# tyt0223/emqx

Measured on AMD Instinct MI355X. Metric: topics matched/sec (node) at 10M filters, 1/2/4/8 GPUs; % HBM roofline, higher is better.
Workload: dtype u32

## Files before the change

### emqx_amd/csrc/egm_ctx.h

```cpp
#pragma once
#include <hip/hip_runtime_api.h>
#include <string.h>

#include <algorithm>
#include <condition_variable>
#include <memory>
#include <mutex>
#include <new>
#include <string>
#include <thread>
#include <unordered_map>
#include <vector>

#include "../../include/emqx_gpu_match.h"
#include "egm_alloc.h"
#include "egm_buf.h"
#include "egm_kernels.h"
#include "egm_table.h"

#pragma GCC visibility push(hidden)
namespace egm {

struct StreamUses {
  std::vector<std::pair<hipStream_t, hipEvent_t>> v;
// ... 15 lines not shown
    }
    v.clear();
  }
};

struct PipeSlot {
  bool busy = false;
  bool waiting = false;
  bool held = false;
  bool sync = false;
  bool abandoned = false;
  uint32_t gen = 0;
  uint32_t n = 0;
  int mode = 0;
  bool want_packed = false;
  bool packed = false;
  uint64_t bytes = 0, maxlen = 0, cap = 0;
  uint64_t o_off = 0;
  PinBuf h_in, h_out, h_stats;
  DevBuf d_in, d_row, d_ids, d_flags, d_row32, d_pk;
  hipEvent_t ev_in = nullptr, ev_match = nullptr, ev_done = nullptr;
  uint64_t epoch = 0;
  uint64_t launch_gen = 0, copied_gen = 0;
  bool copy_failed = false;
  ~PipeSlot() {
    if (ev_in) hipEventDestroy(ev_in);
    if (ev_match) hipEventDestroy(ev_match);
    if (ev_done) hipEventDestroy(ev_done);
  }
};

struct OutLayout {
  size_t o_res, o_row, o_ids, o_fl, o_cnt, total;
};
inline size_t al16(size_t x) { return (x + 15) & ~(size_t)15; }
inline OutLayout out_layout(uint64_t n, uint64_t cap) {
  OutLayout o;
  o.o_res = sizeof(ResultHdr);
  o.o_row = al16(o.o_res + sizeof(egm_result));
  o.o_ids = al16(o.o_row + (n + 1) * 8);
  o.o_fl = al16(o.o_ids + cap * 4);
  o.o_cnt = al16(o.o_fl + n);
  o.total = o.o_cnt + n * 4 + 16;
  return o;
}

struct MatchWs {
  DevBuf wid, lv, tfl, cnt, ids_tmp, pieces, deferred, heavy_stack, tile_sums, stats;
  DevBuf skey, skey_out, sval, order, wfix, sort_tmp;
  DevBuf rec, chunks, dir;
  uint64_t pieces_cap = 0, ids_tmp_cap = 0, rec_cap = 0;
  uint32_t rec_grain = REC_GRAIN, flush_lim = 0;
  uint32_t heavy_cap = 0;
  hipEvent_t ev = nullptr;
  hipStream_t stream = nullptr;
  uint64_t used = 0;
  ~MatchWs() {
    if (ev) hipEventDestroy(ev);
  }
};
constexpr uint32_t MATCH_WORKSPACES = 2;

struct Slot {
  DevBuf nodes, hash_child, edges, dict, dict_blob, dict_off;
  uint64_t n_nodes = 0, n_hc = 0, n_edges = 0, n_dict = 0, n_blob = 0, n_off = 0;
  bool valid = false;
  DirtyLog pending;
  StreamUses uses;
  uint64_t bytes() const {
    return nodes.cap + hash_child.cap + edges.cap + dict.cap + dict_blob.cap + dict_off.cap;
  }
};

struct SubsState {
  bool built = false;
  std::vector<uint64_t> row;
  std::vector<uint32_t> subs;
  std::unordered_map<uint32_t, std::vector<uint32_t>> lists;
  std::unordered_map<uint32_t, uint4> recs;
  std::vector<uint32_t> pending;
  std::vector<uint32_t> stale[2];
  uint64_t tail = 0, garbage = 0;
  int cur = 0;
  StreamUses uses[2];
  uint64_t epoch = 0;
  uint64_t last_appended = 0, last_patched = 0;
  bool last_rebuilt = false;
};

struct Epoch {
  DevTable view{};
  int slot = 0;
  uint64_t id = 0;
  uint64_t n_filters = 0, n_nodes = 0, n_edges = 0, n_words = 0, bytes = 0;
  uint64_t fid_end = 0;
};

struct CommitStats {
  uint64_t h2d = 0, d2d = 0, patched = 0;
  double ms = 0;
};

struct Timing {
  struct Series {
    std::vector<hipEvent_t> ev;
    double ms = 0;
// ... 202 lines not shown
```

### emqx_amd/csrc/egm_kernels.h

```cpp
#pragma once
#include <hip/hip_runtime_api.h>
#include <stdint.h>

#include "egm_common.h"

namespace egm {

struct DevTable {
  const NodeRec* nodes;
  const uint32_t* hash_child;
  const EdgeSlot* edges;
  uint32_t edge_mask;
  const DictSlot* dict;
  uint32_t dict_mask;
  const uint8_t* dict_blob;
  const uint64_t* dict_off;
  uint32_t sig_packed;
};

struct MatchStats {
  unsigned long long cursor;
  unsigned long long visited;
  unsigned long long pieces;
  unsigned long long total_ids;
  unsigned int n_deferred;
  unsigned int heavy_next;
  unsigned int overflow;
  unsigned int errors;
  unsigned int guard;
  unsigned int slow_lanes;
  unsigned long long iters;
  unsigned long long popped;
  unsigned long long bounded;
  unsigned long long lit_probes;
  unsigned long long plus_reads;
  unsigned int n_deep;
  unsigned int slow_iters;
  unsigned long long rec_cursor;
};

constexpr uint32_t REC_HDR = 4;
constexpr uint32_t REC_IDS = REC_HDR + 32;
constexpr uint32_t REC_TAG = 0x5EC0u << 16;
constexpr uint32_t REC_JUMP = 0x4A4Du << 16;
constexpr uint32_t REC_GRAIN = 16384;
constexpr uint32_t REC_DIR = 64;
#ifndef EGM_REC_ALIGN
#define EGM_REC_ALIGN 32
#endif
__host__ __device__ constexpr uint32_t rec_size(uint32_t n_entries) {
  return (REC_IDS + n_entries + (EGM_REC_ALIGN - 1u)) & ~(EGM_REC_ALIGN - 1u);
}
constexpr uint32_t CHUNK_WALKED = 1u;
constexpr uint32_t CHUNK_HEAVY = 2u;

struct MatchWork {
  uint32_t* wid;
  uint32_t* lv;
  uint8_t* tfl;
  uint32_t* cnt;
  uint32_t walk_rows;
  uint32_t ct;
  uint32_t* rec;
  uint64_t rec_cap;
  uint32_t rec_grain;
  uint32_t flush_lim;
  uint4* chunks;
  uint32_t* dir;
  uint32_t* ids_tmp;
  uint64_t ids_cap;
  uint4* pieces;
  uint64_t pieces_cap;
  uint32_t* deferred;
  uint32_t* deep;
  uint4* heavy_stack;
  uint32_t heavy_waves;
  uint32_t heavy_cap;
  uint64_t* tile_sums;
  MatchStats* stats;
  uint32_t debug;
  uint32_t* skey;
  uint32_t* skey_out;
  uint64_t* sval;
  uint64_t* order;
  uint32_t* wfix;
  void* sort_tmp;
  size_t sort_tmp_bytes;
  uint32_t key_shape;
  const uint32_t* n_live;
};

constexpr uint32_t KEY_LEVELS = 4;
constexpr uint32_t FIX_WORDS = 8;
struct WalkOrderOut {
  uint32_t* key;
  uint64_t* val;
  uint32_t* wfix;
  uint32_t shape;
  const uint32_t* n_live;
};

constexpr uint32_t GUARD_STACK = 4u;
constexpr uint32_t GUARD_LOOP = 8u;

constexpr uint32_t DEBUG_FORCE_HEAVY = 1u;
constexpr uint32_t DEBUG_INPUT_ORDER = 4u;
constexpr uint32_t DEBUG_FORCE_GUARD = 8u;

uint32_t walk_key_bits(uint32_t shape);
size_t walk_sort_temp_bytes(uint32_t n, uint32_t shape);
hipError_t launch_walk_sort(uint32_t* keys, uint32_t* keys_tmp, uint64_t* vals, uint64_t* out, void* tmp,
                            MatchStats* stats, uint32_t n, uint32_t kbits, hipStream_t s);

struct MatchOut {
  uint64_t* row_ptr;
  uint32_t* ids;
  uint64_t ids_cap;
  uint32_t* topic;
};
// ... 55 lines not shown
                              hipStream_t s);

hipError_t launch_copy_out(const uint64_t* row, uint32_t n, const uint32_t* ids, uint64_t ids_cap,
                           const uint8_t* flags, uint8_t* h_row, uint8_t* h_ids, uint8_t* h_fl, hipStream_t s,
                           const MatchStats* st = nullptr, MatchStats* h_st = nullptr);

constexpr uint32_t PFX_TOPICS_MAX = 1u << 30;
struct PrefixSlots {
  uint32_t n_ranks, cap_topics;
  uint64_t cap_bytes;
  __host__ __device__ uint64_t off_offsets() const { return 16 + 4ull * cap_topics; }
  __host__ __device__ uint64_t off_bytes() const { return (off_offsets() + 4ull * (cap_topics + 1) + 15) & ~15ull; }
  __host__ __device__ uint64_t slot_bytes() const { return (off_bytes() + cap_bytes + 15) & ~15ull; }
};
hipError_t launch_prefix_route(const uint8_t* blob, const uint32_t* off, uint32_t n, const uint8_t* vpart_rank,
                               uint32_t n_vparts, const PrefixSlots& ps, uint8_t* send, unsigned long long* ctr,
                               uint64_t* dst, hipStream_t s);

hipError_t launch_patch(void* dst, uint32_t rec_bytes, const uint32_t* idx, const void* src, uint64_t n,
                        hipStream_t s);

constexpr uint32_t RN_TERM = 0x80000000u;
constexpr uint32_t RS_SINGLE = 0x80000000u;

struct RetainView {
  const uint4* nodes;
  const uint4* edges;
  uint32_t edge_mask;
  const uint32_t* msg;
  const uint64_t* expiry;
  uint32_t n_topics;
};

struct RetainWork {
  const uint32_t* off;
  const uint32_t* wid;
  const uint32_t* lv;
  const uint8_t* tfl;
  uint32_t* pc;
  uint32_t* paux;
  uint64_t* poff;
  uint64_t* tiles;
  uint32_t *rf, *rlo, *rhi;
  uint32_t* n_ranges;
  uint32_t range_cap;
  uint32_t* alive;
  uint64_t* apre;
  uint32_t* fcnt;
  uint32_t* roff;
  uint64_t now;
  int ge_plain;
};

hipError_t launch_tokenise(const DevTable& tab, const uint8_t* blob, const uint32_t* off, uint32_t n, uint32_t* wid,
                           uint32_t* lv, uint8_t* tfl, hipStream_t s);
hipError_t launch_rs_alive(const RetainView& v, const RetainWork& w, hipStream_t s);
hipError_t launch_rs_init(uint32_t n, uint32_t* pf, uint32_t* pn, hipStream_t s);
hipError_t launch_rs_level(const RetainView& v, const RetainWork& w, uint32_t level, uint32_t np,
                           const uint32_t* pf, const uint32_t* pn, hipStream_t s);
hipError_t launch_rs_fill(const RetainWork& w, uint32_t np, uint64_t nnext, const uint32_t* pf, uint32_t* pf2,
                          uint32_t* pn2, hipStream_t s);
hipError_t launch_rs_rows(const RetainWork& w, uint32_t nr, uint32_t n, uint64_t* row, hipStream_t s);
hipError_t launch_rs_expand(const RetainView& v, const RetainWork& w, uint32_t nr, const uint64_t* row,
                            uint32_t* ids, hipStream_t s);

}
```

### emqx_amd/csrc/egm_kernels.hip

```cpp
#include <hip/hip_runtime.h>

#include <stdio.h>
#include <stdlib.h>
#include <string.h>

#include <algorithm>

#include "egm_kernels.h"

namespace egm {

constexpr int MODE_TRIE = 0;
constexpr int MODE_ROUTES = 1;

constexpr int TOK_BLOCK = 256;
#ifndef EGM_TOK_LDS
#define EGM_TOK_LDS 16256
#endif
constexpr int TOK_LDS = EGM_TOK_LDS;
#ifndef EGM_TOK_WORDS
#define EGM_TOK_WORDS 2528
#endif
constexpr int TOK_WORDS = EGM_TOK_WORDS;
#ifndef EGM_TOK_U
#define EGM_TOK_U 2
#endif
constexpr int TOK_U = EGM_TOK_U;
constexpr int SCAN_TILE = 2048;


__device__ __forceinline__ uint32_t mbcnt(uint64_t m) {
  return __builtin_amdgcn_mbcnt_hi((uint32_t)(m >> 32), __builtin_amdgcn_mbcnt_lo((uint32_t)m, 0u));
}
__device__ __forceinline__ uint32_t popc(uint64_t m) { return (uint32_t)__popcll(m); }

__device__ __forceinline__ void wave_sync() {
  __builtin_amdgcn_fence(__ATOMIC_RELEASE, "wavefront");
  __builtin_amdgcn_s_waitcnt(0xC07F);
  __builtin_amdgcn_wave_barrier();
  __builtin_amdgcn_fence(__ATOMIC_ACQUIRE, "wavefront");
}

__device__ __forceinline__ uint32_t wave_excl_scan(uint32_t v, uint32_t lane, uint32_t* total) {
  uint32_t x = v;
#pragma unroll
  for (int d = 1; d < 64; d <<= 1) {
    uint32_t y = __shfl_up(x, d, 64);
    if (lane >= (uint32_t)d) x += y;
  }
  *total = __shfl(x, 63, 64);
  return x - v;
}

__device__ __forceinline__ uint4 ld16(const void* p) { return *(const uint4*)p; }

__device__ __forceinline__ uint32_t byte_of(uint4 v, uint32_t k) {
  uint32_t w = (k < 8) ? (k < 4 ? v.x : v.y) : (k < 12 ? v.z : v.w);
  return (w >> (8 * (k & 3))) & 0xFFu;
}

__device__ uint32_t dict_probe(const DevTable& tab, uint64_t h, const uint8_t* p, uint32_t len) {
  uint32_t i = (uint32_t)h & tab.dict_mask;
  for (;;) {
    const uint8_t* sp = (const uint8_t*)(tab.dict + i);
    const uint4 a = ld16(sp);
    const uint4 b = ld16(sp + 16);
    if (a.z == NONE) return WID_NONE;
    if (a.x == (uint32_t)h && a.y == (uint32_t)(h >> 32) && a.w == len) {
      bool eq = true;
      if (len <= 16) {
        for (uint32_t k = 0; k < len; ++k) eq &= byte_of(b, k) == p[k];
      } else {
        const uint8_t* q = tab.dict_blob + tab.dict_off[a.z];
        for (uint32_t k = 0; k < len; ++k) eq &= q[k] == p[k];
      }
      if (eq) return a.z;
// ... 53 lines not shown
  const uint32_t x = v ^ 0x2F2F2F2Fu;
  return (x - 0x01010101u) & ~x & 0x80808080u;
}

__device__ __forceinline__ uint32_t byte_range(uint32_t lo, uint32_t hi) {
  const uint32_t a = lo >= 4 ? 0u : (0xFFFFFFFFu << (8 * lo));
  const uint32_t b = hi >= 4 ? 0xFFFFFFFFu : ((1u << (8 * hi)) - 1u);
  return a & b;
}

__device__ __forceinline__ uint32_t dict_resolve(const DevTable& tab, uint64_t h, uint4 a, uint4 b,
                                                 const uint32_t* sw, uint32_t st, uint32_t len) {
  uint32_t i = (uint32_t)h & tab.dict_mask;
  for (;;) {
    if (a.z == NONE) return WID_NONE;
    if (a.x == (uint32_t)h && a.y == (uint32_t)(h >> 32) && a.w == len) {
      bool eq = true;
      if (len <= 16) {
        const uint32_t bw[4] = {b.x, b.y, b.z, b.w};
#pragma unroll
        for (uint32_t k = 0; k < 16; k += 4)
          if (k < len) eq &= low_bytes(lds_word(sw, st + k), len - k) == low_bytes(bw[k >> 2], len - k);
      } else {
        const uint8_t* q = tab.dict_blob + tab.dict_off[a.z];
        for (uint32_t k = 0; k < len; ++k) eq &= q[k] == lds_byte(sw, st + k);
      }
      if (eq) return a.z;
    }
    i = (i + 1) & tab.dict_mask;
    const uint8_t* sp = (const uint8_t*)(tab.dict + i);
    a = ld16(sp);
    b = ld16(sp + 16);
  }
}

__device__ __forceinline__ uint32_t walk_key(const uint32_t* w4, uint32_t D, uint32_t shape) {
  uint64_t h = FNV_BASIS;
  uint32_t k = 0, used = 0;
#pragma unroll
  for (uint32_t l = 0; l < KEY_LEVELS; ++l) {
    const uint32_t bl = (shape >> (4 * l)) & 0xFu;
    h = mix64((h ^ w4[l]) * FNV_PRIME);
    const uint32_t b = (l < D && bl) ? (uint32_t)(h >> (64 - bl)) : 0u;
    k = bl ? ((k << bl) | b) : k;
    used += bl;
  }
  return used < 32 ? k << (32 - used) : k;
}

__device__ __forceinline__ uint64_t sort_val(uint32_t t, uint32_t D, uint32_t f, bool fixed) {
  return (uint64_t)t | ((uint64_t)(min(D, 0xFFFFFFu) | ((f & 0x7Fu) << 24) | (fixed ? 0x80000000u : 0u)) << 32);
}

__global__ __launch_bounds__(TOK_BLOCK) void k_tokenise(DevTable tab, const uint8_t* __restrict__ blob,
                                                        const uint32_t* __restrict__ off, uint32_t n,
                                                        uint32_t* __restrict__ wid, uint32_t* __restrict__ lv,
                                                        uint8_t* __restrict__ tfl, WalkOrderOut wo) {
  __shared__ __attribute__((aligned(16))) uint32_t sw[TOK_LDS / 4 + 1];
  __shared__ uint32_t wpos[TOK_WORDS];
  __shared__ uint8_t wtop[TOK_WORDS];
  __shared__ uint32_t tg[TOK_BLOCK];
  __shared__ uint32_t tex[TOK_BLOCK];
  __shared__ uint32_t tflag[TOK_BLOCK];
  __shared__ uint32_t wsum[TOK_BLOCK / 64];
  const uint32_t blk0 = blockIdx.x * TOK_BLOCK;
  if (blk0 >= n) return;
  const uint32_t tid = threadIdx.x, lane = tid & 63, wv = tid >> 6;
  const uint32_t n_live = wo.n_live ? (wo.n_live[2] ? 0u : min(wo.n_live[0], n)) : n;
  const uint32_t tend = min(blk0 + (uint32_t)TOK_BLOCK, n);
  uint32_t S = TOK_BLOCK;
  for (uint32_t t0 = blk0; t0 < tend;) {
    uint32_t t1, sa, ea;
    for (;;) {
      t1 = min(t0 + S, tend);
      sa = off[t0] & ~3u;
      ea = (off[t1] + 3u) & ~3u;
      if ((ea - sa) <= (uint32_t)TOK_LDS || S == 1) break;
      S >>= 1;
    }
    const uint32_t t = t0 + tid;
    if ((ea - sa) > (uint32_t)TOK_LDS) {
      if (tid == 0) {
        const uint32_t ts = off[t0], len = off[t0 + 1] - ts;
        uint32_t l;
        uint8_t fl;
        tokenise_one(tab, (const uint32_t*)(blob + (ts & ~3u)), ts & 3u, len, ts + t0, wid, &l, &fl);
        if (t0 >= n_live) fl |= TF_SKIP;
        lv[t0] = l;
        tfl[t0] = fl;
        if (wo.key) {
          wo.key[t0] = 0xFFFFFFFFu;
          wo.val[t0] = sort_val(t0, l, fl, false);
        }
      }
      t0 = t1;
      continue;
    }
    {
      const uint32_t nw = (ea - sa) >> 2;
      const uint32_t* src = (const uint32_t*)(blob + sa);
      for (uint32_t i = tid; i < nw; i += TOK_BLOCK) sw[i] = src[i];
    }
    __syncthreads();

    uint32_t ts = 0, len = 0, D = 0, fl = 0;
    if (t < t1) {
      ts = off[t] - sa;
      len = off[t + 1] - off[t];
      uint32_t c = 0;
      for (uint32_t q = ts & ~3u; q < ts + len; q += 4) {
        const uint32_t lo = q < ts ? ts - q : 0u, hi = min(4u, ts + len - q);
        c += popc((uint64_t)(slash_mask(sw[q >> 2]) & byte_range(lo, hi)));
      }
      D = c + 1;
      if (len > 0 && lds_byte(sw, ts) == '$') fl |= TF_DOLLAR;
      if (t >= n_live) fl |= TF_SKIP;
    }
    uint32_t wtot;
    uint32_t ex = wave_excl_scan(D, lane, &wtot);
    if (lane == 0) wsum[wv] = wtot;
    __syncthreads();
    uint32_t W = 0;
#pragma unroll
    for (int k = 0; k < TOK_BLOCK / 64; ++k) {
      if ((uint32_t)k < wv) ex += wsum[k];
      W += wsum[k];
    }
    __syncthreads();
    if (W > (uint32_t)TOK_WORDS) {
      if (S > 1) {
        S >>= 1;
        continue;
      }
      if (tid == 0) {
        uint32_t l;
        uint8_t f;
        tokenise_one(tab, sw, ts, len, off[t] + t, wid, &l, &f);
        if (t >= n_live) f |= TF_SKIP;
        lv[t] = l;
        tfl[t] = f;
        if (wo.key) {
          wo.key[t] = 0xFFFFFFFFu;
          wo.val[t] = sort_val(t, l, f, false);
        }
      }
      __syncthreads();
      t0 = t1;
      continue;
    }
    tflag[tid] = fl | (min(D, 0xFFFFFFu) << 8);

    if (t < t1) {
      const uint32_t g = off[t] + t;
      uint32_t l = 0, ws = ts;
      for (uint32_t q = ts & ~3u; q < ts + len; q += 4) {
        const uint32_t lo = q < ts ? ts - q : 0u, hi = min(4u, ts + len - q);
        uint32_t m = slash_mask(sw[q >> 2]) & byte_range(lo, hi);
        while (m) {
          const uint32_t p = q + (__builtin_ctz(m) >> 3);
          m &= m - 1;
          wpos[ex + l] = ws | ((p - ws) << 16);
          wtop[ex + l] = (uint8_t)tid;
          ++l;
          ws = p + 1;
        }
      }
      wpos[ex + l] = ws | ((ts + len - ws) << 16);
      tex[tid] = ex;
      wtop[ex + l] = (uint8_t)tid;
      tg[tid] = g;
      lv[t] = D;
    }
    __syncthreads();

    for (uint32_t i0 = tid; i0 < W; i0 += TOK_U * TOK_BLOCK) {
      uint32_t st[TOK_U], wl[TOK_U], res[TOK_U];
      uint64_t h[TOK_U];
      bool act[TOK_U], spec[TOK_U];
#pragma unroll
      for (int u = 0; u < TOK_U; ++u) {
        const uint32_t i = i0 + u * TOK_BLOCK;
        act[u] = i < W;
        const uint32_t pw = act[u] ? wpos[i] : 0u;
        st[u] = pw & 0xFFFFu;
        wl[u] = pw >> 16;
        h[u] = lds_word_hash(sw, st[u], wl[u]);
        spec[u] = false;
        res[u] = WID_NONE;
        if (wl[u] == 1) {
          const uint32_t c = lds_byte(sw, st[u]);
          if (c == '+' || c == '#') {
            spec[u] = true;
            res[u] = c == '+' ? WID_PLUS : WID_HASH;
          }
        }
      }
      uint4 a[TOK_U], b[TOK_U];
#pragma unroll
      for (int u = 0; u < TOK_U; ++u) {
        const uint8_t* sp = (const uint8_t*)(tab.dict + ((act[u] && !spec[u]) ? ((uint32_t)h[u] & tab.dict_mask) : 0u));
        a[u] = ld16(sp);
        b[u] = ld16(sp + 16);
      }
#pragma unroll
      for (int u = 0; u < TOK_U; ++u) {
        if (!act[u]) continue;
        const uint32_t i = i0 + u * TOK_BLOCK;
        if (spec[u]) atomicOr(&tflag[wtop[i]], (uint32_t)TF_WILDCARD);
        else res[u] = dict_resolve(tab, h[u], a[u], b[u], sw, st[u], wl[u]);
        if (wo.key) {
          const uint32_t tt = wtop[i], l = i - tex[tt];
          wpos[i] = res[u];
          if ((tflag[tt] >> 8) <= FIX_WORDS) wo.wfix[(uint64_t)(t0 + tt) * FIX_WORDS + l] = res[u];
          else wid[tg[tt] + l] = res[u];
        } else {
          wid[tg[wtop[i]] + i - tex[wtop[i]]] = res[u];
        }
// ... 1278 lines not shown
    s_key[p] = k[i];
    s_val[p] = v[i];
  }
  __syncthreads();
  const uint32_t nt = (uint32_t)min<uint64_t>(SORT_TILE, n - base);
  for (uint32_t j = tid; j < nt; j += SORT_THREADS) {
    const uint32_t kk = s_key[j];
    const uint32_t dg = (kk >> shift) & 0xFFu;
    const uint64_t dst = (uint64_t)s_base[dg] + (j - s_start[dg]);
    if (kout) kout[dst] = kk;
    vout[dst] = s_val[j];
  }
}

static hipError_t walk_sort(const MatchWork& w, uint32_t n, uint32_t kbits, hipStream_t s) {
  const uint32_t begin = 32 - kbits, npass = sort_passes(kbits), tiles = sort_tiles(n);
  uint8_t* tmp = (uint8_t*)w.sort_tmp;
  uint32_t* tickets = (uint32_t*)tmp;
  uint32_t* hist = tickets + SORT_MAX_PASSES;
  uint64_t* vtmp = (uint64_t*)(tmp + SORT_HEAD);
  uint32_t* status = (uint32_t*)(tmp + SORT_HEAD + sort_vals_bytes(n));
  hipError_t e = hipMemsetAsync(tmp, 0, (SORT_MAX_PASSES + SORT_MAX_PASSES * 256) * 4, s);
  if (e != hipSuccess) return e;
  const uint64_t status_words = (uint64_t)npass * tiles * 256;
  const uint32_t hb = (uint32_t)std::min<uint64_t>(SORT_HIST_BLOCKS, std::max<uint64_t>(1, ((uint64_t)n / 4 + 255) / 256));
  hipLaunchKernelGGL(k_sort_hist, dim3(hb), dim3(256), 0, s, w.skey, n, begin, npass, hist, status, status_words);
  for (uint32_t p = 0; p < npass; ++p) {
    const bool last = p + 1 == npass;
    const uint32_t* kin = (p & 1) ? w.skey_out : w.skey;
    uint32_t* kout = last ? nullptr : ((p & 1) ? w.skey : w.skey_out);
    const uint64_t* vin = (p == 0 || !(p & 1)) ? w.sval : vtmp;
    uint64_t* vout = last ? w.order : ((p & 1) ? w.sval : vtmp);
    hipLaunchKernelGGL(k_sort_pass, dim3(tiles), dim3(SORT_THREADS), 0, s, kin, vin, kout, vout, n, begin + 8 * p,
                       hist + 256 * p, status + (uint64_t)p * tiles * 256, tickets + p, w.stats);
  }
  return hipGetLastError();
}

hipError_t launch_walk_sort(uint32_t* keys, uint32_t* keys_tmp, uint64_t* vals, uint64_t* out, void* tmp,
                            MatchStats* stats, uint32_t n, uint32_t kbits, hipStream_t s) {
  if (!n || !kbits || kbits > 32) return hipErrorInvalidValue;
  MatchWork w{};
  w.skey = keys;
  w.skey_out = keys_tmp;
  w.sval = vals;
  w.order = out;
  w.sort_tmp = tmp;
  w.stats = stats;
  return walk_sort(w, n, kbits, s);
}

constexpr uint32_t SORT_MIN_TOPICS = 16384;

hipError_t launch_match(const DevTable& tab, const uint8_t* blob, const uint32_t* off, uint32_t n,
                        int mode, const MatchWork& w_in, const MatchOut& out, hipStream_t s,
                        hipEvent_t* ev_walk, bool* walk_sorted) {
  if (walk_sorted) *walk_sorted = false;
  hipError_t e = hipMemsetAsync(w_in.stats, 0, sizeof(MatchStats), s);
  if (e != hipSuccess) return e;
  if (n == 0) {
    return hipMemsetAsync(out.row_ptr, 0, sizeof(uint64_t), s);
  }
  MatchWork w = w_in;
  w.walk_rows = out.topic != nullptr;
  w.ct = walk_chunk_topics(n);
  const uint32_t kbits = min(walk_key_bits(w.key_shape), 32u);
  const bool sorted = kbits && w.order && n >= SORT_MIN_TOPICS && n < (1u << 29) && !(w.debug & DEBUG_INPUT_ORDER);
  size_t tb = 0;
  if (sorted) {
    tb = walk_sort_temp_bytes(n, w.key_shape);
    if (tb > w.sort_tmp_bytes) return hipErrorInvalidValue;
  }
  WalkOrderOut wo{};
  if (sorted) wo = WalkOrderOut{w.skey, w.sval, w.wfix, w.key_shape, nullptr};
  wo.n_live = w.n_live;
  hipLaunchKernelGGL(k_tokenise, dim3((n + TOK_BLOCK - 1) / TOK_BLOCK), dim3(TOK_BLOCK), 0, s, tab, blob,
                     off, n, w.wid, w.lv, w.tfl, wo);
  trace(s, "k_tokenise");
  if (sorted) {
    e = walk_sort(w, n, kbits, s);
    if (e != hipSuccess) return e;
    if (walk_sorted) *walk_sorted = true;
    trace(s, "walk order sort");
  } else {
    w.order = nullptr;
  }
  if (ev_walk) hipEventRecord(ev_walk[0], s);
  hipLaunchKernelGGL(k_walk<false>, dim3(walk_grid_blocks(n)), dim3(64), 0, s, tab, off, n, mode, w);
  trace(s, "k_walk");
  hipLaunchKernelGGL(k_walk<true>, dim3(deep_grid_blocks(n)), dim3(64), 0, s, tab, off, n, mode, w);
  if (ev_walk) hipEventRecord(ev_walk[1], s);
  trace(s, "k_walk<deep>");
  hipLaunchKernelGGL(k_heavy, dim3(w.heavy_waves), dim3(64), 0, s, tab, off, n, mode, w);
  trace(s, "k_heavy");
  scan_counts(w.cnt, n, w.tile_sums, out.row_ptr, s);
  trace(s, "scan");
  const uint32_t cblocks =
      (uint32_t)std::min<uint64_t>(EGM_COMPACT_BLOCKS, std::max<uint64_t>(256, ((uint64_t)n + 63) / 64));
  const uint32_t rblocks = (uint32_t)std::min<uint64_t>(
      65536, std::max<uint64_t>(1, (((uint64_t)n + w.ct - 1) / w.ct + REC_WAVES - 1) / REC_WAVES));
  hipLaunchKernelGGL(k_rec_burst, dim3(rblocks), dim3(64 * REC_WAVES), 0, s, w.rec, w.rec_cap, w.chunks, w.dir,
                     w.order, n, out.row_ptr, out.topic, out.ids, out.ids_cap, w.stats, w.ct);
  trace(s, "k_rec_burst");
  hipLaunchKernelGGL(k_compact, dim3(cblocks), dim3(64 * COMPACT_WAVES), 0, s, w.pieces, w.ids_tmp, n, out.row_ptr,
                     out.ids, out.ids_cap, w.pieces_cap, w.stats);
  return hipGetLastError();
}

#ifndef EGM_FAN_DS0
#define EGM_FAN_DS0 0
#endif
constexpr uint32_t FAN_CNT_BITS = 24;
constexpr uint32_t FAN_CNT_SAT = (1u << FAN_CNT_BITS) - 1;
constexpr uint32_t FAN_INLINE_ALL = 3;
__device__ __forceinline__ uint64_t rec_start(uint4 r) { return (uint64_t)r.x | ((uint64_t)(r.y & 0xFFu) << 32); }
__device__ __forceinline__ uint32_t rec_count(uint4 r) { return r.y >> 8; }

__global__ __launch_bounds__(256) void k_sub_pairs(const uint64_t* __restrict__ row, const uint32_t* __restrict__ subs,
                                                   uint32_t n_slots, uint4* __restrict__ rp) {
  const uint32_t f = blockIdx.x * 256 + threadIdx.x;
  if (f < n_slots) {
    const uint64_t r0 = row[f], r1 = row[f + 1], c = r1 - r0;
    const uint32_t cs = (uint32_t)min(c, (uint64_t)FAN_CNT_SAT);
    const uint32_t x = c <= FAN_INLINE_ALL ? (c > 2 ? subs[r0 + 2] : 0u) : (uint32_t)r0;
    rp[f] = make_uint4(x, ((uint32_t)(r0 >> 32) & 0xFFu) | (cs << 8), c > 0 ? subs[r0] : 0u, c > 1 ? subs[r0 + 1] : 0u);
  }
}

__global__ __launch_bounds__(256) void k_fan_count(const uint32_t* __restrict__ mids, uint64_t nids,
                                                   SubTable st, uint32_t* __restrict__ wsum,
// ... 605 lines not shown
    uint32_t f = NONE, c = 0;
    if (on) {
      const uint32_t hi = w.rhi[r], lo = w.rlo[r];
      f = w.rf[r];
      c = (hi & RS_SINGLE) ? 1u : (uint32_t)(w.apre[hi] - w.apre[lo]);
    }
    const uint32_t fprev = __shfl_up(f, 1, 64);
    const uint64_t heads = __ballot(lane == 0 || f != fprev);
    const uint32_t seg0 = 63 - __builtin_clzll(heads & ((2ull << lane) - 1));
    uint32_t x = c;
#pragma unroll
    for (int d = 1; d < 64; d <<= 1) {
      const uint32_t y = __shfl_up(x, d, 64);
      if (lane >= seg0 + (uint32_t)d) x += y;
    }
    const uint64_t later = heads & ~((2ull << lane) - 1);
    const uint32_t tail = later ? (uint32_t)__builtin_ctzll(later) - 1 : 63u;
    uint32_t base = 0;
    if (lane == tail && on && x) base = atomicAdd(&w.fcnt[f], x);
    base = __shfl(base, tail, 64);
    if (on) w.roff[r] = base + x - c;
  }
}

__global__ __launch_bounds__(256) void k_rs_expand(RetainView v, RetainWork w, uint32_t nr,
                                                   const uint64_t* __restrict__ row, uint32_t* __restrict__ ids) {
  const uint32_t lane = threadIdx.x & 63;
  const uint32_t nw = gridDim.x * (blockDim.x >> 6);
  for (uint32_t r = blockIdx.x * (blockDim.x >> 6) + (threadIdx.x >> 6); r < nr; r += nw) {
    const uint32_t hr = w.rhi[r], lo = w.rlo[r];
    uint32_t* out = ids + row[w.rf[r]] + w.roff[r];
    if (hr & RS_SINGLE) {
      if (lane == 0) out[0] = v.msg[lo];
      continue;
    }
    const uint64_t a0 = w.apre[lo];
    const uint32_t cnt = (uint32_t)(w.apre[hr] - a0);
    if (cnt == hr - lo) {
      for (uint32_t k = lane; k < cnt; k += 64) out[k] = v.msg[lo + k];
      continue;
    }
    for (uint32_t k = lane; k < cnt; k += 64) {
      uint32_t a = lo, b = hr - 1;
      while (a < b) {
        const uint32_t mid = (a + b) >> 1;
        if (w.apre[mid + 1] > a0 + k) b = mid;
        else a = mid + 1;
      }
      out[k] = v.msg[a];
    }
  }
}

hipError_t launch_tokenise(const DevTable& tab, const uint8_t* blob, const uint32_t* off, uint32_t n, uint32_t* wid,
                           uint32_t* lv, uint8_t* tfl, hipStream_t s) {
  const WalkOrderOut none{};
  if (!n) return hipSuccess;
  hipLaunchKernelGGL(k_tokenise, dim3((n + TOK_BLOCK - 1) / TOK_BLOCK), dim3(TOK_BLOCK), 0, s, tab, blob, off, n,
                     wid, lv, tfl, none);
  return hipGetLastError();
}

static uint32_t grid_for(uint64_t n, uint32_t cap = 8192) {
  return (uint32_t)std::max<uint64_t>(1, std::min<uint64_t>((n + 255) / 256, cap));
}

hipError_t launch_rs_alive(const RetainView& v, const RetainWork& w, hipStream_t s) {
  if (v.n_topics) {
    hipLaunchKernelGGL(k_rs_alive, dim3(grid_for(v.n_topics)), dim3(256), 0, s, v.expiry, v.n_topics, w.now, w.alive);
  }
  scan_counts(w.alive, v.n_topics, w.tiles, w.apre, s);
  return hipGetLastError();
}

hipError_t launch_rs_init(uint32_t n, uint32_t* pf, uint32_t* pn, hipStream_t s) {
  if (n) hipLaunchKernelGGL(k_rs_init, dim3(grid_for(n)), dim3(256), 0, s, n, pf, pn);
  return hipGetLastError();
}

hipError_t launch_rs_level(const RetainView& v, const RetainWork& w, uint32_t level, uint32_t np,
                           const uint32_t* pf, const uint32_t* pn, hipStream_t s) {
  hipLaunchKernelGGL(k_rs_step, dim3(grid_for(np)), dim3(256), 0, s, v, w, level, np, pf, pn);
  scan_counts(w.pc, np, w.tiles, w.poff, s);
  return hipGetLastError();
}

hipError_t launch_rs_fill(const RetainWork& w, uint32_t np, uint64_t nnext, const uint32_t* pf, uint32_t* pf2,
                          uint32_t* pn2, hipStream_t s) {
  if (nnext) hipLaunchKernelGGL(k_rs_fill, dim3(grid_for(nnext)), dim3(256), 0, s, w, np, nnext, pf, pf2, pn2);
  return hipGetLastError();
}

hipError_t launch_rs_rows(const RetainWork& w, uint32_t nr, uint32_t n, uint64_t* row, hipStream_t s) {
  hipError_t e = hipMemsetAsync(w.fcnt, 0, ((size_t)n + 1) * 4, s);
  if (e != hipSuccess) return e;
  if (nr) hipLaunchKernelGGL(k_rs_count, dim3(grid_for(nr)), dim3(256), 0, s, w, nr);
  scan_counts(w.fcnt, n, w.tiles, row, s);
  return hipGetLastError();
}

hipError_t launch_rs_expand(const RetainView& v, const RetainWork& w, uint32_t nr, const uint64_t* row,
                            uint32_t* ids, hipStream_t s) {
  if (nr)
    hipLaunchKernelGGL(k_rs_expand, dim3(std::min<uint32_t>((nr + 3) / 4, 16384)), dim3(256), 0, s, v, w, nr, row,
                       ids);
  return hipGetLastError();
}

}
```

### emqx_amd/csrc/egm_match.cpp

```cpp
#include <stdlib.h>

#include "egm_ctx.h"

using namespace egm;

constexpr uint32_t WALK_KEY_DEFAULT = 0x7764u;
static uint32_t walk_key_shape() {
  const char* v = getenv("EGM_WALK_KEY");
  const uint32_t shape = (v && *v) ? (uint32_t)strtoul(v, nullptr, 16) & 0xFFFFu : WALK_KEY_DEFAULT;
  return walk_key_bits(shape) <= 32 ? shape : WALK_KEY_DEFAULT;
}

static uint64_t walk_sort_min_bytes() {
  const char* v = getenv("EGM_WALK_SORT_MIN_BYTES");
  return (v && *v) ? strtoull(v, nullptr, 10) : (1ull << 30);
}

static uint32_t env_u32(const char* name, uint32_t dflt, uint32_t lo, uint32_t hi) {
  const char* v = getenv(name);
  if (!v || !*v) return dflt;
  const long long k = atoll(v);
  return (uint32_t)std::min<long long>(std::max<long long>(k, lo), hi);
}
static uint32_t flush_lim() { return env_u32("EGM_FLUSH_AT", walk_stage(), 1, walk_stage()); }
static uint32_t rec_grain() { return env_u32("EGM_REC_SEG", REC_GRAIN, 64, 1u << 24) & ~(uint32_t)(EGM_REC_ALIGN - 1); }

MatchWs& egm::pick_ws(egm_ctx* c, hipStream_t s) {
  uint32_t k = 0;
  for (uint32_t i = 0; i < MATCH_WORKSPACES; ++i) {
    if (c->ws[i].stream == s && c->ws[i].used) {
      k = i;
      break;
    }
    if (c->ws[i].used < c->ws[k].used) k = i;
  }
  MatchWs& W = c->ws[k];
  if (W.used && W.stream != s && W.ev) hipStreamWaitEvent(s, W.ev, 0);
  c->cur_ws = k;
  W.used = ++c->ws_clock;
  return W;
}

int egm::ensure_work(egm_ctx* c, MatchWs& W, uint32_t n, uint64_t blob_bytes, uint64_t ids_cap,
                     uint64_t max_levels) {
  hipError_t e;
  const uint64_t nn = (uint64_t)n + 1;
  if ((e = W.wid.ensure((blob_bytes + nn) * 4)) != hipSuccess) return c->hip_fail(e, "wid");
  if ((e = W.lv.ensure(nn * 4)) != hipSuccess) return c->hip_fail(e, "lv");
  if ((e = W.tfl.ensure(nn)) != hipSuccess) return c->hip_fail(e, "tfl");
  if ((e = W.cnt.ensure(nn * 4)) != hipSuccess) return c->hip_fail(e, "cnt");
  W.flush_lim = flush_lim();
  W.rec_grain = rec_grain();
  const uint64_t rcap = rec_capacity(ids_cap, n, W.flush_lim, W.rec_grain);
  if ((e = W.rec.ensure(rcap * 4)) != hipSuccess) return c->hip_fail(e, "flush records");
  W.rec_cap = W.rec.cap / 4;
  if (W.rec_cap >= (1ull << 34)) return c->fail(EGM_E_INVAL, "batch too large: > 16G u32 of flush records (split it)");
  if ((e = W.chunks.ensure(walk_chunk_cap(n) * 16)) != hipSuccess) return c->hip_fail(e, "chunk records");
  if ((e = W.dir.ensure(walk_chunk_cap(n) * REC_DIR * 4)) != hipSuccess)
    return c->hip_fail(e, "chunk directories");
  const uint64_t tcap = ids_cap + 4096;
  if (tcap >= 0xFFFFFFF0ull) return c->fail(EGM_E_INVAL, "batch too large: > 4G matched ids (split it)");
  if ((e = W.ids_tmp.ensure(tcap * 4)) != hipSuccess) return c->hip_fail(e, "ids_tmp");
  W.ids_tmp_cap = W.ids_tmp.cap / 4;
  if ((e = W.pieces.ensure(((uint64_t)n + 4096) * 16)) != hipSuccess) return c->hip_fail(e, "pieces");
  W.pieces_cap = std::min<uint64_t>(W.pieces.cap / 16, 0xFFFFFFF0ull);
  if ((e = W.deferred.ensure(walk_chunk_cap(n) * 4 * 2)) != hipSuccess) return c->hip_fail(e, "deferred");
  const uint32_t hcap = heavy_stack_items(max_levels);
  if ((e = W.heavy_stack.ensure((uint64_t)c->heavy_waves * hcap * 16)) != hipSuccess)
    return c->hip_fail(e, "heavy stack");
  W.heavy_cap = (uint32_t)std::min<uint64_t>(W.heavy_stack.cap / 16 / c->heavy_waves, 0xFFFFFFFFull);
  if ((e = W.tile_sums.ensure((scan_tiles(n) + 2) * 8)) != hipSuccess) return c->hip_fail(e, "tile_sums");
  if ((e = W.stats.ensure(sizeof(MatchStats))) != hipSuccess) return c->hip_fail(e, "stats");
  const uint32_t shape = walk_key_shape();
  if (shape) {
    if ((e = W.skey.ensure(nn * 4)) != hipSuccess) return c->hip_fail(e, "sort keys");
    if ((e = W.skey_out.ensure(nn * 4)) != hipSuccess) return c->hip_fail(e, "sort keys");
    if ((e = W.sval.ensure(nn * 8)) != hipSuccess) return c->hip_fail(e, "sort values");
    if ((e = W.order.ensure(nn * 8)) != hipSuccess) return c->hip_fail(e, "walk order");
    if ((e = W.wfix.ensure(nn * 4 * FIX_WORDS)) != hipSuccess) return c->hip_fail(e, "fixed-stride words");

    if ((e = W.sort_tmp.ensure(walk_sort_temp_bytes(n, shape))) != hipSuccess) return c->hip_fail(e, "sort scratch");
  }
  if (!W.ev && (e = hipEventCreateWithFlags(&W.ev, hipEventDisableTiming)) != hipSuccess)
    return c->hip_fail(e, "workspace event");
  return EGM_OK;
}

static MatchWork work_view(egm_ctx* c, MatchWs& W) {
  MatchWork w{};
  w.wid = W.wid.as<uint32_t>();
  w.lv = W.lv.as<uint32_t>();
  w.tfl = W.tfl.as<uint8_t>();
  w.cnt = W.cnt.as<uint32_t>();
  w.rec = W.rec.as<uint32_t>();
  w.rec_cap = W.rec_cap;
  w.rec_grain = W.rec_grain;
  w.flush_lim = W.flush_lim;
  w.chunks = W.chunks.as<uint4>();
  w.dir = W.dir.as<uint32_t>();
  w.ids_tmp = W.ids_tmp.as<uint32_t>();
  w.ids_cap = W.ids_tmp_cap;
  w.pieces = W.pieces.as<uint4>();
  w.pieces_cap = W.pieces_cap;
  w.deferred = W.deferred.as<uint32_t>();
  w.deep = w.deferred + W.deferred.cap / 8;
  w.heavy_stack = W.heavy_stack.as<uint4>();
  w.heavy_waves = c->heavy_waves;
  w.heavy_cap = W.heavy_cap;
  w.tile_sums = W.tile_sums.as<uint64_t>();
  w.stats = W.stats.as<MatchStats>();
  w.debug = c->debug;
  w.key_shape = walk_key_shape();
  if (w.key_shape && W.order.p) {
    w.skey = W.skey.as<uint32_t>();
    w.skey_out = W.skey_out.as<uint32_t>();
    w.sval = W.sval.as<uint64_t>();
    w.order = W.order.as<uint64_t>();
    w.wfix = W.wfix.as<uint32_t>();

    w.sort_tmp = W.sort_tmp.p;
    w.sort_tmp_bytes = W.sort_tmp.cap;
  } else {
    w.key_shape = 0;
  }

  return w;
}

int egm::run_match(egm_ctx* c, MatchWs& W, const Epoch& ep, const uint8_t* d_blob, const uint32_t* d_off, uint32_t n,
                   int mode, hipStream_t s, uint64_t* d_row, uint32_t* d_ids, uint64_t ids_cap,
                   const uint32_t* d_n_live, uint32_t* d_topic) {
  MatchWork w = work_view(c, W);
  w.n_live = d_n_live;
  if (ep.bytes < walk_sort_min_bytes()) w.key_shape = 0;
  MatchOut o{d_row, d_ids, ids_cap, d_topic};
  hipEvent_t evs[2] = {nullptr, nullptr};
  hipEvent_t* evp = c->timing.take_pair(evs);
  bool walk_sorted = false;
  hipError_t e = launch_match(ep.view, d_blob, d_off, n, mode, w, o, s, evp, &walk_sorted);
  c->last_walk.order = (walk_sorted && !d_topic) ? w.order : nullptr;
  c->last_walk.row = d_row;
  c->last_walk.n = n;
  c->last_walk.ws = (uint32_t)(&W - c->ws);
  c->slots[ep.slot].uses.note(s);
  c->timing.push_pair(c->timing.walk, evp);
  if (e != hipSuccess) return c->hip_fail(e, "launch_match");
  c->last_pending = true;
  c->last_stream = s;
  return EGM_OK;
}
// ... 159 lines not shown
```

### emqx_amd/csrc/egm_retain.cpp

```cpp
#include <hip/hip_runtime_api.h>
#include <stdlib.h>
#include <string.h>

#include <algorithm>
#include <mutex>
#include <numeric>
#include <string>
#include <unordered_map>
#include <vector>

#include "../../include/emqx_gpu_match.h"
#include "egm_alloc.h"
#include "egm_buf.h"
#include "egm_kernels.h"

using namespace egm;

namespace {

template <class T>
hipError_t put_vec(DevBuf& b, const std::vector<T>& v) {
  hipError_t e = b.ensure(v.size() * sizeof(T) + 16);
  if (e == hipSuccess && !v.empty()) e = hipMemcpy(b.p, v.data(), v.size() * sizeof(T), hipMemcpyHostToDevice);
  return e;
// ... 279 lines not shown
int egm_rstore_commit(egm_rstore* r) {
  if (!r) return EGM_E_INVAL;
  std::lock_guard<std::mutex> g(r->mu);
  if (hipSetDevice(r->device) != hipSuccess) return EGM_E_DEVICE;
  return rs_commit_locked(r);
}

int egm_rstore_match(egm_rstore* r, const uint8_t* blob, const uint32_t* off, uint32_t n, uint64_t now_ms, int mode,
                     egm_result** out) {
  if (!r || !out || (mode != EGM_RMODE_MATCH && mode != EGM_RMODE_DISPATCH)) return EGM_E_INVAL;
  if (n && !off) return EGM_E_INVAL;
  for (uint32_t i = 0; i < n; ++i)
    if (off[i + 1] < off[i]) return EGM_E_INVAL;
  if (n && !blob && off[n] > off[0]) return EGM_E_INVAL;
  *out = nullptr;
  std::lock_guard<std::mutex> g(r->mu);
  if (hipSetDevice(r->device) != hipSuccess) return EGM_E_DEVICE;
  int rc = rs_commit_locked(r);
  if (rc) return rc;
  hipStream_t s = r->stream;
  hipError_t e;
  const uint32_t base0 = n ? off[0] : 0;
  const uint64_t bytes = n ? (uint64_t)off[n] - base0 : 0;
  std::vector<uint32_t> loff(n + 1);
  for (uint32_t i = 0; i <= n; ++i) loff[i] = n ? off[i] - base0 : 0;
  const uint32_t M = r->view.n_topics;
  const size_t nn = (size_t)n + 1;
  if ((e = r->in_blob.ensure(bytes + 16)) || (e = r->in_off.ensure(nn * 4)) ||
      (e = r->wid.ensure((bytes + nn) * 4)) || (e = r->lv.ensure(nn * 4)) || (e = r->tfl.ensure(nn)) ||
      (e = r->alive.ensure(((size_t)M + 1) * 4)) || (e = r->apre.ensure(((size_t)M + 2) * 8)) ||
      (e = r->fcnt.ensure(nn * 4)) || (e = r->row.ensure(nn * 8)) || (e = r->nr.ensure(16)))
    return r->hip_fail(e, "retained workspace");
  if (bytes && (e = hipMemcpyAsync(r->in_blob.p, blob + base0, bytes, hipMemcpyHostToDevice, s)))
    return r->hip_fail(e, "H2D filters");
  if ((e = hipMemcpyAsync(r->in_off.p, loff.data(), nn * 4, hipMemcpyHostToDevice, s)))
    return r->hip_fail(e, "H2D offsets");

  RetainWork w{};
  w.off = r->in_off.as<uint32_t>();
  w.wid = r->wid.as<uint32_t>();
  w.lv = r->lv.as<uint32_t>();
  w.tfl = r->tfl.as<uint8_t>();
  w.alive = r->alive.as<uint32_t>();
  w.apre = r->apre.as<uint64_t>();
  w.fcnt = r->fcnt.as<uint32_t>();
  w.n_ranges = r->nr.as<uint32_t>();
  w.now = now_ms;
  w.ge_plain = mode == EGM_RMODE_DISPATCH;
  auto tiles_for = [&](uint64_t m) { return (scan_tiles((uint32_t)std::min<uint64_t>(m, 0xFFFFFFFFull)) + 2) * 8; };
  size_t tiles_need = std::max(tiles_for(M), tiles_for(n));
  if ((e = r->tiles.ensure(tiles_need))) return r->hip_fail(e, "tiles");
  w.tiles = r->tiles.as<uint64_t>();

  if ((e = launch_tokenise(r->dtab, r->in_blob.as<uint8_t>(), w.off, n, r->wid.as<uint32_t>(), r->lv.as<uint32_t>(),
                           r->tfl.as<uint8_t>(), s)) ||
      (e = launch_rs_alive(r->view, w, s)))
    return r->hip_fail(e, "tokenise/alive");

  uint64_t range_cap = std::max<uint64_t>(4 * (uint64_t)n + 1024, r->rf.cap / 4);
  uint32_t n_ranges = 0;
  for (int attempt = 0; attempt < 2; ++attempt) {
    if (range_cap > 0xFFFFFFF0ull) return r->fail(EGM_E_NOMEM, "too many result ranges in one batch");
    if ((e = r->rf.ensure(range_cap * 4)) || (e = r->rlo.ensure(range_cap * 4)) || (e = r->rhi.ensure(range_cap * 4)) ||
        (e = r->roff.ensure(range_cap * 4)))
      return r->hip_fail(e, "ranges");
    w.rf = r->rf.as<uint32_t>();
    w.rlo = r->rlo.as<uint32_t>();
    w.rhi = r->rhi.as<uint32_t>();
    w.roff = r->roff.as<uint32_t>();
    w.range_cap = (uint32_t)range_cap;
    if ((e = hipMemsetAsync(w.n_ranges, 0, 4, s))) return r->hip_fail(e, "memset");
    uint64_t np = n;
    int cur = 0;
    if ((e = r->pf[0].ensure(nn * 4)) || (e = r->pn[0].ensure(nn * 4))) return r->hip_fail(e, "frontier");
    if ((e = launch_rs_init(n, r->pf[0].as<uint32_t>(), r->pn[0].as<uint32_t>(), s)))
      return r->hip_fail(e, "init");
    for (uint32_t level = 0; np; ++level) {
      if (np > 0xFFFFFFF0ull) return r->fail(EGM_E_NOMEM, "frontier too large (split the batch)");
      if ((e = r->pc.ensure((np + 1) * 4)) || (e = r->paux.ensure((np + 1) * 4)) ||
          (e = r->poff.ensure((np + 2) * 8)) || (e = r->tiles.ensure(std::max(tiles_need, tiles_for(np)))))
        return r->hip_fail(e, "level workspace");
      w.pc = r->pc.as<uint32_t>();
      w.paux = r->paux.as<uint32_t>();
      w.poff = r->poff.as<uint64_t>();
      w.tiles = r->tiles.as<uint64_t>();
      if ((e = launch_rs_level(r->view, w, level, (uint32_t)np, r->pf[cur].as<uint32_t>(), r->pn[cur].as<uint32_t>(),
                               s)))
        return r->hip_fail(e, "level");
      uint64_t nnext = 0;
      if ((e = hipMemcpyAsync(&nnext, w.poff + np, 8, hipMemcpyDeviceToHost, s)) || (e = hipStreamSynchronize(s)))
        return r->hip_fail(e, "level readback");
      if (nnext) {
        if ((e = r->pf[cur ^ 1].ensure(nnext * 4 + 16)) || (e = r->pn[cur ^ 1].ensure(nnext * 4 + 16)))
          return r->hip_fail(e, "frontier");
        if ((e = launch_rs_fill(w, (uint32_t)np, nnext, r->pf[cur].as<uint32_t>(), r->pf[cur ^ 1].as<uint32_t>(),
                                r->pn[cur ^ 1].as<uint32_t>(), s)))
          return r->hip_fail(e, "fill");
        if ((e = hipStreamSynchronize(s))) return r->hip_fail(e, "fill sync");
      }
      cur ^= 1;
      np = nnext;
    }
    if ((e = hipMemcpyAsync(&n_ranges, w.n_ranges, 4, hipMemcpyDeviceToHost, s)) || (e = hipStreamSynchronize(s)))
      return r->hip_fail(e, "ranges readback");
    if (n_ranges <= range_cap) break;
    range_cap = (uint64_t)n_ranges + n_ranges / 4 + 1024;
    if (attempt == 1) return r->fail(EGM_E_NOMEM, "ranges capacity");
// ... 43 lines not shown
```

Before: 1.257 billion.

## Size tokenise LDS dynamically by mean topic length and cache slash bitmasks

Moves the tokenise kernel's LDS staging buffers to dynamic shared memory. A smaller shape is picked when the mean topic length is short, so six blocks fit per CU instead of five. The first pass now also packs per-topic slash positions into two 64-bit masks, so the word-extraction pass can skip rescanning LDS for topics up to 128 bytes. The cost is extra registers, more batch splitting for larger batches under the small shape, and a getenv call on every launch.

Measured after the change: 1.274 billion (median of 6 runs). +1.4%, better.

```diff
diff --git a/emqx_amd/csrc/egm_ctx.h b/emqx_amd/csrc/egm_ctx.h
--- a/emqx_amd/csrc/egm_ctx.h
+++ b/emqx_amd/csrc/egm_ctx.h
@@ -91,6 +91,7 @@
   uint64_t pieces_cap = 0, ids_tmp_cap = 0, rec_cap = 0;
   uint32_t rec_grain = REC_GRAIN, flush_lim = 0;
   uint32_t heavy_cap = 0;
+  uint64_t blob_bytes = 0;
   hipEvent_t ev = nullptr;
   hipStream_t stream = nullptr;
   uint64_t used = 0;
diff --git a/emqx_amd/csrc/egm_kernels.h b/emqx_amd/csrc/egm_kernels.h
--- a/emqx_amd/csrc/egm_kernels.h
+++ b/emqx_amd/csrc/egm_kernels.h
@@ -65,6 +65,7 @@
   uint64_t rec_cap;
   uint32_t rec_grain;
   uint32_t flush_lim;
+  uint64_t blob_bytes;
   uint4* chunks;
   uint32_t* dir;
   uint32_t* ids_tmp;
@@ -226,8 +227,8 @@
   int ge_plain;
 };
 
-hipError_t launch_tokenise(const DevTable& tab, const uint8_t* blob, const uint32_t* off, uint32_t n, uint32_t* wid,
-                           uint32_t* lv, uint8_t* tfl, hipStream_t s);
+hipError_t launch_tokenise(const DevTable& tab, const uint8_t* blob, uint64_t nbytes, const uint32_t* off, uint32_t n,
+                           uint32_t* wid, uint32_t* lv, uint8_t* tfl, hipStream_t s);
 hipError_t launch_rs_alive(const RetainView& v, const RetainWork& w, hipStream_t s);
 hipError_t launch_rs_init(uint32_t n, uint32_t* pf, uint32_t* pn, hipStream_t s);
 hipError_t launch_rs_level(const RetainView& v, const RetainWork& w, uint32_t level, uint32_t np,
diff --git a/emqx_amd/csrc/egm_kernels.hip b/emqx_amd/csrc/egm_kernels.hip
--- a/emqx_amd/csrc/egm_kernels.hip
+++ b/emqx_amd/csrc/egm_kernels.hip
@@ -14,14 +14,22 @@
 constexpr int MODE_ROUTES = 1;
 
 constexpr int TOK_BLOCK = 256;
-#ifndef EGM_TOK_LDS
-#define EGM_TOK_LDS 16256
-#endif
-constexpr int TOK_LDS = EGM_TOK_LDS;
-#ifndef EGM_TOK_WORDS
-#define EGM_TOK_WORDS 2528
-#endif
-constexpr int TOK_WORDS = EGM_TOK_WORDS;
+struct TokShape {
+  uint32_t bytes;
+  uint32_t words;
+  uint32_t mean_max;
+};
+constexpr TokShape TOK_SHAPES[] = {
+    {12288, 2296, 40},
+    {16256, 2528, 0xFFFFFFFFu},
+};
+constexpr int TOK_N_SHAPES = sizeof(TOK_SHAPES) / sizeof(TOK_SHAPES[0]);
+constexpr uint32_t TOK_STATIC_LDS = 3 * 256 * 4 + 256 / 64 * 4;
+constexpr uint32_t tok_dyn_lds(const TokShape& sh) { return sh.bytes + 4 + sh.words * 5; }
+constexpr uint32_t tok_granules(const TokShape& sh) { return (TOK_STATIC_LDS + tok_dyn_lds(sh) + 1279) / 1280; }
+static_assert(tok_granules(TOK_SHAPES[0]) * 6 * 1280 <= 163840, "shape 0: 6 blocks per CU");
+static_assert(tok_granules(TOK_SHAPES[1]) * 5 * 1280 <= 163840, "shape 1: 5 blocks per CU");
+static_assert(TOK_SHAPES[0].bytes % 4 == 0 && TOK_SHAPES[1].bytes % 4 == 0 && TOK_SHAPES[1].bytes < 65536, "wpos layout");
 #ifndef EGM_TOK_U
 #define EGM_TOK_U 2
 #endif
@@ -181,13 +189,16 @@
   return (uint64_t)t | ((uint64_t)(min(D, 0xFFFFFFu) | ((f & 0x7Fu) << 24) | (fixed ? 0x80000000u : 0u)) << 32);
 }
 
-__global__ __launch_bounds__(TOK_BLOCK) void k_tokenise(DevTable tab, const uint8_t* __restrict__ blob,
+extern __shared__ __attribute__((aligned(16))) uint32_t tok_lds[];
+
+__global__ __launch_bounds__(TOK_BLOCK, 6) void k_tokenise(DevTable tab, const uint8_t* __restrict__ blob,
                                                         const uint32_t* __restrict__ off, uint32_t n,
                                                         uint32_t* __restrict__ wid, uint32_t* __restrict__ lv,
-                                                        uint8_t* __restrict__ tfl, WalkOrderOut wo) {
-  __shared__ __attribute__((aligned(16))) uint32_t sw[TOK_LDS / 4 + 1];
-  __shared__ uint32_t wpos[TOK_WORDS];
-  __shared__ uint8_t wtop[TOK_WORDS];
+                                                        uint8_t* __restrict__ tfl, WalkOrderOut wo,
+                                                        uint32_t cap_bytes, uint32_t cap_words) {
+  uint32_t* const sw = tok_lds;
+  uint32_t* const wpos = sw + (cap_bytes >> 2) + 1;
+  uint8_t* const wtop = (uint8_t*)(wpos + cap_words);
   __shared__ uint32_t tg[TOK_BLOCK];
   __shared__ uint32_t tex[TOK_BLOCK];
   __shared__ uint32_t tflag[TOK_BLOCK];
@@ -204,11 +215,11 @@
       t1 = min(t0 + S, tend);
       sa = off[t0] & ~3u;
       ea = (off[t1] + 3u) & ~3u;
-      if ((ea - sa) <= (uint32_t)TOK_LDS || S == 1) break;
+      if ((ea - sa) <= cap_bytes || S == 1) break;
       S >>= 1;
     }
     const uint32_t t = t0 + tid;
-    if ((ea - sa) > (uint32_t)TOK_LDS) {
+    if ((ea - sa) > cap_bytes) {
       if (tid == 0) {
         const uint32_t ts = off[t0], len = off[t0 + 1] - ts;
         uint32_t l;
@@ -233,13 +244,18 @@
     __syncthreads();
 
     uint32_t ts = 0, len = 0, D = 0, fl = 0;
+    uint64_t sl0 = 0, sl1 = 0;
     if (t < t1) {
       ts = off[t] - sa;
       len = off[t + 1] - off[t];
-      uint32_t c = 0;
-      for (uint32_t q = ts & ~3u; q < ts + len; q += 4) {
+      uint32_t c = 0, j = 0;
+      for (uint32_t q = ts & ~3u; q < ts + len; q += 4, j += 4) {
         const uint32_t lo = q < ts ? ts - q : 0u, hi = min(4u, ts + len - q);
-        c += popc((uint64_t)(slash_mask(sw[q >> 2]) & byte_range(lo, hi)));
+        const uint32_t m = slash_mask(sw[q >> 2]) & byte_range(lo, hi);
+        c += popc((uint64_t)m);
+        const uint64_t nib = (((m >> 7) * 0x00204081u) >> 21) & 0xFu;
+        if (j < 64) sl0 |= nib << j;
+        else if (j < 128) sl1 |= nib << (j - 64);
       }
       D = c + 1;
       if (len > 0 && lds_byte(sw, ts) == '$') fl |= TF_DOLLAR;
@@ -256,7 +272,7 @@
       W += wsum[k];
     }
     __syncthreads();
-    if (W > (uint32_t)TOK_WORDS) {
+    if (W > cap_words) {
       if (S > 1) {
         S >>= 1;
         continue;
@@ -282,16 +298,23 @@
     if (t < t1) {
       const uint32_t g = off[t] + t;
       uint32_t l = 0, ws = ts;
-      for (uint32_t q = ts & ~3u; q < ts + len; q += 4) {
-        const uint32_t lo = q < ts ? ts - q : 0u, hi = min(4u, ts + len - q);
-        uint32_t m = slash_mask(sw[q >> 2]) & byte_range(lo, hi);
-        while (m) {
-          const uint32_t p = q + (__builtin_ctz(m) >> 3);
-          m &= m - 1;
-          wpos[ex + l] = ws | ((p - ws) << 16);
-          wtop[ex + l] = (uint8_t)tid;
-          ++l;
-          ws = p + 1;
+      auto word_ends = [&](uint32_t p) {
+        wpos[ex + l] = ws | ((p - ws) << 16);
+        wtop[ex + l] = (uint8_t)tid;
+        ++l;
+        ws = p + 1;
+      };
+      if ((ts & 3u) + len <= 128) {
+        for (; sl0; sl0 &= sl0 - 1) word_ends((ts & ~3u) + (uint32_t)__builtin_ctzll(sl0));
+        for (; sl1; sl1 &= sl1 - 1) word_ends((ts & ~3u) + 64 + (uint32_t)__builtin_ctzll(sl1));
+      } else {
+        for (uint32_t q = ts & ~3u; q < ts + len; q += 4) {
+          const uint32_t lo = q < ts ? ts - q : 0u, hi = min(4u, ts + len - q);
+          uint32_t m = slash_mask(sw[q >> 2]) & byte_range(lo, hi);
+          while (m) {
+            word_ends(q + (__builtin_ctz(m) >> 3));
+            m &= m - 1;
+          }
         }
       }
       wpos[ex + l] = ws | ((ts + len - ws) << 16);
@@ -1676,6 +1699,21 @@
 
 constexpr uint32_t SORT_MIN_TOPICS = 16384;
 
+static const TokShape& tok_shape(uint64_t nbytes, uint32_t n) {
+  const char* v = getenv("EGM_TOK_SHAPE");
+  if (v && *v >= '0' && *v < '0' + TOK_N_SHAPES && !v[1]) return TOK_SHAPES[*v - '0'];
+  int k = 0;
+  while (k + 1 < TOK_N_SHAPES && nbytes > (uint64_t)TOK_SHAPES[k].mean_max * n) ++k;
+  return TOK_SHAPES[k];
+}
+
+static void launch_k_tokenise(const DevTable& tab, const uint8_t* blob, uint64_t nbytes, const uint32_t* off, uint32_t n,
+                              uint32_t* wid, uint32_t* lv, uint8_t* tfl, const WalkOrderOut& wo, hipStream_t s) {
+  const TokShape& sh = tok_shape(nbytes, n);
+  hipLaunchKernelGGL(k_tokenise, dim3((n + TOK_BLOCK - 1) / TOK_BLOCK), dim3(TOK_BLOCK), tok_dyn_lds(sh), s, tab, blob,
+                     off, n, wid, lv, tfl, wo, sh.bytes, sh.words);
+}
+
 hipError_t launch_match(const DevTable& tab, const uint8_t* blob, const uint32_t* off, uint32_t n,
                         int mode, const MatchWork& w_in, const MatchOut& out, hipStream_t s,
                         hipEvent_t* ev_walk, bool* walk_sorted) {
@@ -1698,8 +1736,7 @@
   WalkOrderOut wo{};
   if (sorted) wo = WalkOrderOut{w.skey, w.sval, w.wfix, w.key_shape, nullptr};
   wo.n_live = w.n_live;
-  hipLaunchKernelGGL(k_tokenise, dim3((n + TOK_BLOCK - 1) / TOK_BLOCK), dim3(TOK_BLOCK), 0, s, tab, blob,
-                     off, n, w.wid, w.lv, w.tfl, wo);
+  launch_k_tokenise(tab, blob, w.blob_bytes, off, n, w.wid, w.lv, w.tfl, wo, s);
   trace(s, "k_tokenise");
   if (sorted) {
     e = walk_sort(w, n, kbits, s);
@@ -2411,12 +2448,11 @@
   }
 }
 
-hipError_t launch_tokenise(const DevTable& tab, const uint8_t* blob, const uint32_t* off, uint32_t n, uint32_t* wid,
-                           uint32_t* lv, uint8_t* tfl, hipStream_t s) {
+hipError_t launch_tokenise(const DevTable& tab, const uint8_t* blob, uint64_t nbytes, const uint32_t* off, uint32_t n,
+                           uint32_t* wid, uint32_t* lv, uint8_t* tfl, hipStream_t s) {
   const WalkOrderOut none{};
   if (!n) return hipSuccess;
-  hipLaunchKernelGGL(k_tokenise, dim3((n + TOK_BLOCK - 1) / TOK_BLOCK), dim3(TOK_BLOCK), 0, s, tab, blob, off, n,
-                     wid, lv, tfl, none);
+  launch_k_tokenise(tab, blob, nbytes, off, n, wid, lv, tfl, none, s);
   return hipGetLastError();
 }
 
diff --git a/emqx_amd/csrc/egm_match.cpp b/emqx_amd/csrc/egm_match.cpp
--- a/emqx_amd/csrc/egm_match.cpp
+++ b/emqx_amd/csrc/egm_match.cpp
@@ -45,6 +45,7 @@
                      uint64_t max_levels) {
   hipError_t e;
   const uint64_t nn = (uint64_t)n + 1;
+  W.blob_bytes = blob_bytes;
   if ((e = W.wid.ensure((blob_bytes + nn) * 4)) != hipSuccess) return c->hip_fail(e, "wid");
   if ((e = W.lv.ensure(nn * 4)) != hipSuccess) return c->hip_fail(e, "lv");
   if ((e = W.tfl.ensure(nn)) != hipSuccess) return c->hip_fail(e, "tfl");
@@ -96,6 +97,7 @@
   w.rec_cap = W.rec_cap;
   w.rec_grain = W.rec_grain;
   w.flush_lim = W.flush_lim;
+  w.blob_bytes = W.blob_bytes;
   w.chunks = W.chunks.as<uint4>();
   w.dir = W.dir.as<uint32_t>();
   w.ids_tmp = W.ids_tmp.as<uint32_t>();
diff --git a/emqx_amd/csrc/egm_retain.cpp b/emqx_amd/csrc/egm_retain.cpp
--- a/emqx_amd/csrc/egm_retain.cpp
+++ b/emqx_amd/csrc/egm_retain.cpp
@@ -355,7 +355,7 @@
   if ((e = r->tiles.ensure(tiles_need))) return r->hip_fail(e, "tiles");
   w.tiles = r->tiles.as<uint64_t>();
 
-  if ((e = launch_tokenise(r->dtab, r->in_blob.as<uint8_t>(), w.off, n, r->wid.as<uint32_t>(), r->lv.as<uint32_t>(),
+  if ((e = launch_tokenise(r->dtab, r->in_blob.as<uint8_t>(), bytes, w.off, n, r->wid.as<uint32_t>(), r->lv.as<uint32_t>(),
                            r->tfl.as<uint8_t>(), s)) ||
       (e = launch_rs_alive(r->view, w, s)))
     return r->hip_fail(e, "tokenise/alive");
```
